# dangvansam/viet-asr

Hardware: AMD Instinct MI355X
Metric: real_time_factor (higher is better)
Workload: dtype f32 via 2xf16 split operands (22-bit significands, 3 f16 MFMA products per multiply, fp32 accumulate); 1 GPU; BASELINE configs[2]: quartznet15x5 greedy CTC, batch=64x10s 16kHz mono per GPU, wav in HBM -> collapsed ids; batch_per_gpu=64, parallelism=utterance-shard x1

## Files before the change

include/vasr_devtools.h:

```cpp
#ifndef VASR_DEVTOOLS_H_
#define VASR_DEVTOOLS_H_
#include "vasr.h"
#ifdef __cplusplus
extern "C" {
#endif

VASR_API int vasr_profile_bracket_overhead(vasr_stream stream, int n, double* out_us);
VASR_API int vasr_fused_tile_choice(int64_t tiles128, int compute_units);
VASR_API int vasr_bench_depthwise(const float* d_x, const float* d_w, const int32_t* d_lens, int batch, int channels,
                         int64_t frames, int kernel, float* d_y, vasr_stream stream);
VASR_API int vasr_bench_depthwise_layer(const float* d_x, const float* d_w, const int32_t* d_lens_in, const int32_t* d_lens_out,
                               int batch, int channels, int64_t frames_in, int kernel, int stride, int dilation, float* d_y,
                               uint32_t* d_amax, int amax_stride, vasr_stream stream);
VASR_API int vasr_depthwise_mfma_table_size(int kernel, int dilation);
VASR_API int vasr_pack_depthwise_taps(const float* h_w, int channels, int kernel, int dilation, uint32_t* h_table, float* h_inv);
VASR_API int vasr_bench_depthwise_mfma(const float* d_x, const uint32_t* d_taps, const float* d_tap_inv, const int32_t* d_lens,
                              int batch, int channels, int64_t frames, int kernel, int dilation, float* d_y,
                              uint32_t* d_amax, int amax_stride, vasr_stream stream);
VASR_API int vasr_pack_pointwise(const float* h_w, int cout, int cin, int m_pad, float* h_out);
VASR_API int vasr_conv_gemm_weights(const float* h_w, int cout, int cin, int kernel, float* h_out);
VASR_API int vasr_bench_pointwise(const float* d_x, const float* d_wt, const float* d_scale, const float* d_shift,
                         int batch, int cin, int cout, int64_t frames, float* d_y, vasr_stream stream);

VASR_API int vasr_bench_mfma_sustained(int gemm_mode, int workgroups, int steps, float* d_sink, double* flops, vasr_stream stream);

VASR_API int vasr_pack_pointwise_f16x2(const float* h_w, int cout, int cin, int m_pad, uint16_t* h_out, float* inv_scale);
VASR_API int vasr_bench_pointwise_f16x2(const float* d_x, const uint16_t* d_w16, float w_inv_scale, const float* d_scale,
                               const float* d_shift, int batch, int cin, int cout, int64_t frames, float* d_y,
                               uint32_t* d_amax, int amax_stride, vasr_stream stream);

VASR_API int vasr_pack_pointwise_bf16x3(const float* h_w, int cout, int cin, int m_pad, uint16_t* h_out);
// ... 11 lines not shown
```

viet-asr_amd/_lib.py:

```python
import ctypes as C
import os

import numpy as np
import torch

_HERE = os.path.dirname(os.path.abspath(__file__))
LIB_PATH = os.environ.get("VASR_LIB_PATH") or os.path.join(_HERE, "lib", "libvasr_hip.so")
DEV_LIB_PATH = os.environ.get("VASR_LIB_PATH") or os.path.join(_HERE, "lib", "libvasr_hip_dev.so")


class VasrError(RuntimeError):
    pass


class BlockDesc(C.Structure):
    _fields_ = [(n, C.c_int32) for n in
                ("filters", "repeat", "kernel", "stride", "dilation", "residual", "separable", "residual_dense")]


class FrontendDesc(C.Structure):
    _fields_ = [("sample_rate", C.c_int32), ("n_fft", C.c_int32), ("win_length", C.c_int32),
                ("hop_length", C.c_int32), ("n_mels", C.c_int32), ("preemph", C.c_float),
                ("log_guard", C.c_float), ("normalize", C.c_int32),
                ("h_window", C.POINTER(C.c_float)), ("h_filterbank", C.POINTER(C.c_float)),
# ... 59 lines not shown
                                 C.c_float, C.c_float, C.POINTER(_P)]),
    "vasr_lm_destroy": (None, [_P]),
    "vasr_beam_workgroups": (C.c_int, [C.c_int]),
    "vasr_beam_hash_init": (C.c_uint64, []),
    "vasr_beam_hash_step": (C.c_uint64, [C.c_uint64, C.c_uint64]),
    "vasr_last_error": (C.c_char_p, []),
    "vasr_version": (C.c_char_p, []),
    "vasr_abi_version": (C.c_int, []),
    "vasr_algorithmic_work": (C.c_int, [_P, C.c_int, C.c_int64, C.POINTER(C.c_double)]),
    "vasr_profile_begin": (C.c_int, [_P]),
    "vasr_profile_end": (C.c_int, [_P, C.POINTER(C.c_double), C.POINTER(C.c_int64), C.POINTER(C.c_double), C.POINTER(C.c_double)]),
    "vasr_padded_frames": (C.c_int64, [C.c_int64]),
}

DEV_SIGNATURES = {
    "vasr_pack_pointwise_f16x2": (C.c_int, [_P, C.c_int, C.c_int, C.c_int, _P, C.POINTER(C.c_float)]),
    "vasr_bench_pointwise_f16x2": (C.c_int, [_P, _P, C.c_float, _P, _P, C.c_int, C.c_int, C.c_int, C.c_int64, _P, _P,
                                             C.c_int, _P]),
    "vasr_depthwise_mfma_table_size": (C.c_int, [C.c_int, C.c_int]),
    "vasr_pack_depthwise_taps": (C.c_int, [_P, C.c_int, C.c_int, C.c_int, _P, _P]),
    "vasr_bench_depthwise_mfma": (C.c_int, [_P, _P, _P, _P, C.c_int, C.c_int, C.c_int64, C.c_int, C.c_int, _P, _P, C.c_int, _P]),
    "vasr_profile_bracket_overhead": (C.c_int, [_P, C.c_int, C.POINTER(C.c_double)]),
    "vasr_fused_tile_choice": (C.c_int, [C.c_int64, C.c_int]),
    "vasr_pack_pointwise": (C.c_int, [_P, C.c_int, C.c_int, C.c_int, _P]),
    "vasr_conv_gemm_weights": (C.c_int, [_P, C.c_int, C.c_int, C.c_int, _P]),
    "vasr_pack_pointwise_bf16x3": (C.c_int, [_P, C.c_int, C.c_int, C.c_int, _P]),
    "vasr_bench_pointwise_bf16x3": (C.c_int, [_P, _P, _P, _P, C.c_int, C.c_int, C.c_int, C.c_int64, _P, _P]),
    "vasr_bench_mfma_sustained": (C.c_int, [C.c_int, C.c_int, C.c_int, _P, C.POINTER(C.c_double), _P]),
    "vasr_bench_depthwise": (C.c_int, [_P, _P, _P, C.c_int, C.c_int, C.c_int64, C.c_int, _P, _P]),
    "vasr_bench_depthwise_layer": (C.c_int, [_P, _P, _P, _P, C.c_int, C.c_int, C.c_int64, C.c_int, C.c_int, C.c_int, _P, _P,
                                             C.c_int, _P]),
    "vasr_bench_pointwise": (C.c_int, [_P, _P, _P, _P, C.c_int, C.c_int, C.c_int, C.c_int64, _P, _P]),
    "vasr_bench_groupnorm": (C.c_int, [_P, _P, C.c_int, C.c_int, C.c_int64, C.c_int, C.c_int, _P, _P, C.c_int, _P, _P]),
}

ABI_VERSION = 8

_lib = None
_dev = None


def _load(path, tables):
    if not os.path.exists(path):
        raise VasrError(
            f"{path} is missing: build it with `python -c 'import __graft_entry__ as g; g.build()'` "
            "(or `make -C viet-asr_amd/csrc`). There is no CPU fallback for this path.")
# ... 167 lines not shown
```

viet-asr_amd/csrc/encoder_fused.hip:

```cpp
#include <cstdlib>

#include "vasr_internal.h"
#include "vasr_device.h"
#include <type_traits>

namespace vasr {

namespace {

constexpr int FC = 256;
constexpr int FCH = 64;
constexpr int FNT = 512;

template <int BN>
struct FTile {
  static_assert(BN == 128 || BN == 64, "tile width");
  static constexpr int FPS = BN / 8;
  static constexpr int NT = BN / 32;
  static constexpr int KHS = BN == 128 ? 3 : 2;
  static constexpr int kBimgBytes = 2 * 2 * 4 * 2 * BN * 16;
  static constexpr int kWPitch = BN == 128 ? 1664 : 1152;
  static constexpr int kWWave = 8 * kWPitch;
  static constexpr int kWinBytes = 4 * kWWave;
  static constexpr int kSegBytes = FPS * 8 + 16;
};

template <int K, int BN>
struct FGeom {
  using TL = FTile<BN>;
  static constexpr int FPS = TL::FPS;
  static constexpr int PAD = K / 2;
  static constexpr int PADL = (PAD + 3) & ~3;
  static constexpr int OFF = PADL - PAD;
  static constexpr int W = (PADL + BN + (K - 1 - PAD) + 3) & ~3;
  static constexpr int W4 = W / 4;
  static constexpr int NLD = (8 * W4 + 63) / 64;
  static constexpr int NF = OFF + FPS - 1 + K;
  static constexpr int NR = (NF + 1) / 2;
  static constexpr int KP = (K + 2) & ~1;
  static constexpr int TB = 8;
  static constexpr int NB = (K + TB - 1) / TB;
  static constexpr int kTapBytes = (FC / 2) * KP * 8;
  static constexpr size_t LDS = (size_t)TL::kBimgBytes + TL::kWinBytes + kTapBytes;
  static_assert(W * 8 + ((W + FPS - 1) / FPS) * 16 <= TL::kWPitch, "window row does not fit its pitch");
  static_assert(FPS * 7 + 2 * NR <= W, "a lane's reads leave the window");
  static_assert(NLD >= FPS / 4, "the residual rows of a lane use the staging registers of the window items");
  static_assert(LDS <= 163840, "LDS budget");
  static constexpr int qend(int blk) {
    const int k1 = TB * (blk + 1) < K ? TB * (blk + 1) : K;
    return (OFF + k1 + FPS - 1 + 1) / 2;
  }
};

struct FusedArgs {
  const float* x;
  int64_t ldx;
  const int32_t* lens_in;
  const int32_t* lens_out;
  const float* taps;
  float dw_l1;
  AmaxTab amax_x;
  const uint4* wt;
  float w_inv_scale;
  const float* scale;
  const float* shift;
  float* y;
  int64_t ldy;
  int32_t frames;
  int32_t relu;
  int32_t act;
  AmaxTab amax_y;
  const int32_t* lens_y;
  const float* x2;
  int64_t ldx2;
  const int32_t* lens2;
  AmaxTab amax_x2;
  int32_t batch;
};

__device__ __forceinline__ void lds_barrier() { asm volatile("s_waitcnt lgkmcnt(0)\n\ts_barrier" ::: "memory"); }

template <int BN>
__device__ __forceinline__ int bimg_slot(int n, int kh) { return (n & ~15) | ((n & 15) ^ ((n >> 4) | (kh << FTile<BN>::KHS))); }
template <int BN>
__device__ __forceinline__ constexpr int bimg_off(int buf, int plane, int ks) { return (((buf * 2 + plane) * 4 + ks) * 2) * BN * 16; }

template <int K, bool DUAL, int BN, int EPI = 0>
__global__ __launch_bounds__(FNT, 1) void dwpw_fused_kernel(FusedArgs a, int tiles_t, int n_blocks) {
  using G = FGeom<K, BN>;
  using TL = FTile<BN>;
  constexpr int FPS = TL::FPS, NT = TL::NT, kWPitch = TL::kWPitch, kWWave = TL::kWWave;
  extern __shared__ __attribute__((aligned(16))) unsigned char smem[];
  unsigned char* bimg = smem;
  unsigned char* wins = smem + TL::kBimgBytes;
  unsigned char* tapl = smem + TL::kBimgBytes + TL::kWinBytes;

  const int bid = xcd_remap(blockIdx.x, n_blocks);
  const int b = bid / tiles_t;
  const int tile = bid % tiles_t;
  const int t0 = tile * BN;
  const int tid = threadIdx.x, lane = tid & 63;
  const int wave = __builtin_amdgcn_readfirstlane(tid >> 6);
  const int len_in = a.lens_in[b], len_out = a.lens_out[b];
  const int len2 = DUAL ? a.lens2[b] : 0;
  constexpr int NCH = (DUAL ? 2 : 1) * (FC / FCH);

  const int zf = max(len_out, DUAL ? len2 : 0);
  const bool live = t0 < zf;

  float xs = 1.f, out_scale = 1.f;
  unsigned amv[8], amv2[8];
  if (live) {
    amax_request(a.amax_x.p, a.amax_x.stride, a.amax_x.n, b, lane, amv);
    if (DUAL) amax_request(a.amax_x2.p, a.amax_x2.stride, a.amax_x2.n, b, lane, amv2);
  }
  constexpr int kTapV4 = G::kTapBytes / 16, kTapIt = (kTapV4 + FNT - 1) / FNT;
  auto tap_copy = [&]() {
    v4f tv[kTapIt];
#pragma unroll
    for (int i = 0; i < kTapIt; ++i) {
      const int idx = tid + i * FNT;
      tv[i] = reinterpret_cast<const v4f*>(a.taps)[idx < kTapV4 ? idx : kTapV4 - 1];
    }
#pragma unroll
    for (int i = 0; i < kTapIt; ++i) {
      const int idx = tid + i * FNT;
      if (idx < kTapV4) reinterpret_cast<v4f*>(tapl)[idx] = tv[i];
    }
  };

  if (wave < 4) {
    const int kh = lane >> 5, l31 = lane & 31;
    const int wm = wave * 64;
    constexpr int ksteps = NCH * 4;
    const uint4* __restrict__ ap = a.wt + ((int64_t)(wm / 32) * ksteps) * 2 * 64 + lane;
    const int64_t a_tile = (int64_t)ksteps * 2 * 64;
    f32x16 acc[2][NT];
#pragma unroll
    for (int i = 0; i < 2; ++i)
#pragma unroll
      for (int j = 0; j < NT; ++j)
#pragma unroll
        for (int r = 0; r < 16; ++r) acc[i][j][r] = 0.f;
    if (live) {
      int boff[NT];
#pragma unroll
      for (int j = 0; j < NT; ++j) boff[j] = (kh * BN + bimg_slot<BN>(32 * j + l31, kh)) * 16;
      uint4 aw[4][2][2];
      auto aload = [&](int s, uint4 (&dst)[2][2]) {
        const int sc = s < ksteps ? s : ksteps - 1;
#pragma unroll
        for (int i = 0; i < 2; ++i)
#pragma unroll
          for (int p = 0; p < 2; ++p) dst[i][p] = ap[i * a_tile + ((int64_t)sc * 2 + p) * 64];
      };
      aload(0, aw[0]);
      aload(1, aw[1]);
      aload(2, aw[2]);
      tap_copy();
      {
        unsigned mx = amax_collect(a.amax_x.p, a.amax_x.stride, a.amax_x.n, b, lane, amv);
        mx = __float_as_uint(__uint_as_float(mx) * a.dw_l1);
        if (DUAL) mx = max(mx, amax_collect(a.amax_x2.p, a.amax_x2.stride, a.amax_x2.n, b, lane, amv2));
        float inv;
        f16_scale(mx, &xs, &inv);
        out_scale = inv * a.w_inv_scale;
      }
      lds_barrier();
#pragma unroll 1
      for (int c = 0; c < NCH; c += 2) {
#pragma unroll
        for (int cc = 0; cc < 2; ++cc) {
          lds_barrier();
          uint4 bf[3][2];
#pragma unroll
          for (int p = 0; p < 2; ++p) {
            bf[0][p] = *reinterpret_cast<const uint4*>(bimg + bimg_off<BN>(cc, p, 0) + boff[0]);
            bf[1][p] = *reinterpret_cast<const uint4*>(bimg + bimg_off<BN>(cc, p, 1 / NT) + boff[1 % NT]);
          }
#pragma unroll
          for (int s = 0; s < 4; ++s) {
            const int gs = (c + cc) * 4 + s;
            aload(gs + 3, aw[(s + 3) % 4]);
            __builtin_amdgcn_sched_barrier(0);
            uint4 (&cw)[2][2] = aw[s];
#pragma unroll
            for (int j = 0; j < NT; ++j) {
              const int g = s * NT + j, cur_f = g % 3, nxt_f = (g + 2) % 3;
              if (g + 2 < 4 * NT) {
#pragma unroll
                for (int p = 0; p < 2; ++p)
                  bf[nxt_f][p] = *reinterpret_cast<const uint4*>(bimg + bimg_off<BN>(cc, p, (g + 2) / NT) + boff[(g + 2) % NT]);
              }
              __builtin_amdgcn_sched_barrier(0);
#pragma unroll
              for (int i = 0; i < 2; ++i)
                acc[i][j] = __builtin_amdgcn_mfma_f32_32x32x16_f16(__builtin_bit_cast(f16x8, cw[i][1]), __builtin_bit_cast(f16x8, bf[cur_f][0]), acc[i][j], 0, 0, 0);
#pragma unroll
              for (int i = 0; i < 2; ++i)
                acc[i][j] = __builtin_amdgcn_mfma_f32_32x32x16_f16(__builtin_bit_cast(f16x8, cw[i][0]), __builtin_bit_cast(f16x8, bf[cur_f][1]), acc[i][j], 0, 0, 0);
#pragma unroll
              for (int i = 0; i < 2; ++i)
                acc[i][j] = __builtin_amdgcn_mfma_f32_32x32x16_f16(__builtin_bit_cast(f16x8, cw[i][0]), __builtin_bit_cast(f16x8, bf[cur_f][0]), acc[i][j], 0, 0, 0);
            }
          }
        }
      }
    }
    AmaxTracker amax{a.amax_y.p ? (a.lens_y ? a.lens_y[b] : a.frames) : 0};
    const Epilogue<EPI> epi(a.relu, a.act, 0);
    float* stage = reinterpret_cast<float*>(wins + wave * kWWave);
    v4f scv[2][4], shv[2][4];
#pragma unroll
    for (int i = 0; i < 2; ++i)
#pragma unroll
      for (int q = 0; q < 4; ++q) {
        scv[i][q] = *reinterpret_cast<const v4f*>(a.scale + wm + i * 32 + 8 * q + 4 * kh);
        shv[i][q] = *reinterpret_cast<const v4f*>(a.shift + wm + i * 32 + 8 * q + 4 * kh);
      }
#pragma unroll
    for (int i = 0; i < 2; ++i) {
#pragma unroll
      for (int q = 0; q < 4; ++q) {
        float* buf = stage + ((i * 4 + q) & 1) * (8 * BN);
        const int mq = wm + i * 32 + 8 * q;
        const v4f sc = scv[i][q], sh = shv[i][q];
        wave_fence();
#pragma unroll
        for (int rr = 0; rr < 4; ++rr)
#pragma unroll
          for (int j = 0; j < NT; ++j)
            buf[(4 * kh + rr) * BN + 32 * j + l31] = fmaf(acc[i][j][4 * q + rr] * out_scale, sc[rr], sh[rr]);
        wave_fence();
        v4f pv[NT];
#pragma unroll
        for (int k = 0; k < NT; ++k) {
          const int f = lane + 64 * k, row = f / (BN / 4), c4 = f % (BN / 4);
          pv[k] = *reinterpret_cast<const v4f*>(buf + row * BN + 4 * c4);
        }
#pragma unroll
        for (int k = 0; k < NT; ++k) {
          const int f = lane + 64 * k, row = f / (BN / 4), c4 = f % (BN / 4);
          const int m = mq + row, t = t0 + 4 * c4;
          const v4f v = epi.apply4(pv[k]);
          *reinterpret_cast<v4f*>(a.y + ((int64_t)b * FC + m) * a.ldy + t) = v;
          amax.track4(v, t);
        }
      }
    }
    if (a.amax_y.p) amax_publish(a.amax_y.p, a.amax_y.stride, b, tile * 4 + wave, amax.ymax, lane);
    return;
  }

  if (!live) return;
  const int pw = wave - 4;
  const int p = lane >> 3, s = lane & 7;
  unsigned char* win = wins + pw * kWWave;
  auto item = [&](int j, int& sp, int& q) { const int idx = lane + 64 * j; sp = idx / G::W4; q = idx - sp * G::W4; };
  v4f st[G::NLD][2];
  auto gload_dw = [&](int c) {
    const float* xb = a.x + ((int64_t)b * FC + c * FCH + pw * 16) * a.ldx;
#pragma unroll
    for (int j = 0; j < G::NLD; ++j) {
      int sp, q;
      item(j, sp, q);
      sp = sp < 8 ? sp : 7;
      int t = t0 - G::PADL + 4 * q;
      t = t < 0 ? 0 : (t > (int)a.ldx - 4 ? (int)a.ldx - 4 : t);
      const float* r0 = xb + (int64_t)(2 * sp) * a.ldx + t;
      st[j][0] = *reinterpret_cast<const v4f*>(r0);
      st[j][1] = *reinterpret_cast<const v4f*>(r0 + a.ldx);
    }
  };
  auto gload_x2 = [&](int c) {
    const float* xb = a.x2 + ((int64_t)b * FC + (c - FC / FCH) * FCH + pw * 16 + 2 * p) * a.ldx2 + t0 + FPS * s;
#pragma unroll
    for (int j = 0; j < FPS / 4; ++j) {
      st[j][0] = *reinterpret_cast<const v4f*>(xb + 4 * j);
      st[j][1] = *reinterpret_cast<const v4f*>(xb + a.ldx2 + 4 * j);
    }
  };
  gload_dw(0);
  tap_copy();
  {
    unsigned mx = amax_collect(a.amax_x.p, a.amax_x.stride, a.amax_x.n, b, lane, amv);
    mx = __float_as_uint(__uint_as_float(mx) * a.dw_l1);
    if (DUAL) mx = max(mx, amax_collect(a.amax_x2.p, a.amax_x2.stride, a.amax_x2.n, b, lane, amv2));
    float inv;
    f16_scale(mx, &xs, &inv);
  }
  lds_barrier();

  const int kh = p >> 2;
  const int wbase = (kh * BN) * 16 + 4 * (p & 3);
  const int nsw = (FPS * s) & ~15;
  const int sx = (((FPS * s) & 15) ^ (((FPS * s) >> 4) | (kh << TL::KHS))) << 4;
  auto emit = [&](int buf, const v2f (&d)[FPS], int nvalid) {
#pragma unroll
    for (int j = 0; j < FPS; ++j) {
      const float sj = j < nvalid ? xs : 0.f;
      const v2f v = {d[j].x * sj, d[j].y * sj};
      const f16x2 hv = __builtin_convertvector(v, f16x2);
      const v2f r = v - __builtin_convertvector(hv, v2f);
      const f16x2 lv = __builtin_convertvector(r, f16x2);
      const int off = wbase + ((nsw << 4) | ((j << 4) ^ sx));
      *reinterpret_cast<unsigned*>(bimg + bimg_off<BN>(buf, 0, 0) + pw * (2 * BN * 16) + off) = __builtin_bit_cast(unsigned, hv);
      *reinterpret_cast<unsigned*>(bimg + bimg_off<BN>(buf, 1, 0) + pw * (2 * BN * 16) + off) = __builtin_bit_cast(unsigned, lv);
    }
  };

  const unsigned char* rd = win + p * kWPitch + TL::kSegBytes * s;
  const int nvalid = len_out - (t0 + FPS * s);
#pragma unroll 1
  for (int c = 0; c < FC / FCH; c += 2) {
#pragma unroll
    for (int cc = 0; cc < 2; ++cc) {
      const int ch = c + cc;
#pragma unroll
      for (int j = 0; j < G::NLD; ++j) {
        int sp, q;
        item(j, sp, q);
        const int t = t0 - G::PADL + 4 * q;
        v4f u = st[j][0], w = st[j][1];
#pragma unroll
        for (int e = 0; e < 4; ++e) {
          const bool ok = (unsigned)(t + e) < (unsigned)len_in;
          u[e] = ok ? u[e] : 0.f;
          w[e] = ok ? w[e] : 0.f;
        }
        if (sp < 8) {
          unsigned char* dst = win + sp * kWPitch + (4 * q) * 8 + ((4 * q) / FPS) * 16;
          *reinterpret_cast<v4f*>(dst) = v4f{u.x, w.x, u.y, w.y};
          *reinterpret_cast<v4f*>(dst + 16) = v4f{u.z, w.z, u.w, w.w};
        }
      }
      wave_fence();
      if (ch + 1 < FC / FCH) gload_dw(ch + 1);
      else if (DUAL) gload_x2(FC / FCH);
      const unsigned char* tp = tapl + ((ch * FCH + pw * 16) / 2 + p) * (G::KP * 8);
      v2f xw[2 * G::NR];
      auto load_units = [&](int qa, int qb) {
#pragma unroll
        for (int qq = qa; qq < qb; ++qq) {
          const v4f v = *reinterpret_cast<const v4f*>(rd + qq * 16 + (qq / (FPS / 2)) * 16);
          xw[2 * qq] = v.xy;
          xw[2 * qq + 1] = v.zw;
        }
      };
      v2f acc[FPS];
#pragma unroll
      for (int j = 0; j < FPS; ++j) acc[j] = v2f{0.f, 0.f};
      load_units(0, G::qend(0));
      v2f wn[G::TB];
      auto load_taps = [&](int blk) {
#pragma unroll
        for (int k2 = 0; k2 < G::TB / 2; ++k2) {
          if (G::TB * blk + 2 * k2 < G::KP) {
            const v4f v = *reinterpret_cast<const v4f*>(tp + (G::TB * blk + 2 * k2) * 8);
            wn[2 * k2] = v.xy;
            wn[2 * k2 + 1] = v.zw;
          }
        }
// ... 21 lines not shown
      lds_barrier();
    }
  }
  if constexpr (DUAL) {
    const int nv2 = len2 - (t0 + FPS * s);
#pragma unroll 1
    for (int c = FC / FCH; c < NCH; c += 2) {
#pragma unroll
      for (int cc = 0; cc < 2; ++cc) {
        const int ch = c + cc;
        v2f d[FPS];
#pragma unroll
        for (int j = 0; j < FPS / 4; ++j)
#pragma unroll
          for (int e = 0; e < 4; ++e) d[4 * j + e] = v2f{st[j][0][e], st[j][1][e]};
        if (ch + 1 < NCH) gload_x2(ch + 1);
        emit(cc, d, nv2);
        lds_barrier();
      }
    }
  }
}

template <int K, bool DUAL, int BN>
int launch_fused_t(const FusedArgs& a, hipStream_t st, int* amax_n) {
  using G = FGeom<K, BN>;
  const int tiles_t = (int)(a.ldy / BN);
  const int n_blocks = tiles_t * a.batch;
  if (a.amax_y.p) {
    if (tiles_t * 4 > a.amax_y.stride) return (int)hipErrorInvalidValue;
    if (amax_n) *amax_n = tiles_t * 4;
  }
  const int epi = epilogue_kind(a.relu, a.act, false);
  auto kern = epi == 2 ? dwpw_fused_kernel<K, DUAL, BN, 2> : epi == 1 ? dwpw_fused_kernel<K, DUAL, BN, 1> : dwpw_fused_kernel<K, DUAL, BN, 0>;
  static std::atomic<uint64_t> lds_opted[3];
  const hipError_t attr = dyn_lds_opt_in(reinterpret_cast<const void*>(kern), (int)G::LDS, lds_opted[epi]);
  if (attr != hipSuccess) return (int)attr;
  VASR_LAUNCH(kern, dim3(n_blocks), dim3(FNT), G::LDS, st, a, tiles_t, n_blocks);
  return 0;
}

}

bool fused_dwpw_supported(int channels, int cout, int kernel, int stride, int dilation) {
  return channels == FC && cout == FC && stride == 1 && dilation == 1 && (kernel == 33 || kernel == 39);
}
int fused_dwpw_taps_per_pair(int kernel) { return (kernel + 2) & ~1; }

float pack_fused_taps(const float* w, int channels, int kernel, float* out) {
  const int kp = fused_dwpw_taps_per_pair(kernel);
  float l1 = 0.f;
  for (int c = 0; c < channels; ++c) {
    double s = 0;
    for (int k = 0; k < kernel; ++k) s += std::fabs((double)w[(size_t)c * kernel + k]);
    l1 = (float)s > l1 ? (float)s : l1;
  }
  for (int pr = 0; pr < channels / 2; ++pr)
    for (int k = 0; k < kp; ++k)
      for (int h = 0; h < 2; ++h)
        out[((size_t)pr * kp + k) * 2 + h] = k < kernel ? w[(size_t)(2 * pr + h) * kernel + k] : 0.f;
  return __builtin_nextafterf(l1, 3.0e38f);
}

int launch_fused_dwpw(const FusedLaunch& f, hipStream_t st, int* amax_n) {
  FusedArgs a{};
  a.x = f.x; a.ldx = f.ldx; a.lens_in = f.lens_in; a.lens_out = f.lens_out; a.taps = f.taps; a.dw_l1 = f.dw_l1;
  a.amax_x = f.amax_x; a.wt = reinterpret_cast<const uint4*>(f.wt); a.w_inv_scale = f.w_inv_scale; a.scale = f.scale;
  a.shift = f.shift; a.y = f.y; a.ldy = f.ldy; a.frames = f.frames; a.relu = f.relu; a.act = f.act; a.amax_y = f.amax_y;
  a.lens_y = f.lens_y; a.x2 = f.x2; a.ldx2 = f.ldx2; a.lens2 = f.lens2; a.amax_x2 = f.amax_x2; a.batch = f.batch;
  const bool dual = f.x2 != nullptr;
  if (f.tile_cols == 64) {
    if (f.kernel == 33) return dual ? launch_fused_t<33, true, 64>(a, st, amax_n) : launch_fused_t<33, false, 64>(a, st, amax_n);
    if (f.kernel == 39) return dual ? launch_fused_t<39, true, 64>(a, st, amax_n) : launch_fused_t<39, false, 64>(a, st, amax_n);
    return -1;
  }
  if (f.kernel == 33) return dual ? launch_fused_t<33, true, 128>(a, st, amax_n) : launch_fused_t<33, false, 128>(a, st, amax_n);
  if (f.kernel == 39) return dual ? launch_fused_t<39, true, 128>(a, st, amax_n) : launch_fused_t<39, false, 128>(a, st, amax_n);
  return -1;
}

}
```

viet-asr_amd/csrc/vasr_api.cpp:

```cpp
#include <hip/hip_runtime.h>

#include <cmath>
#include <cstdarg>
#include <cstdio>
#include <cstdlib>
#include <cstring>
#include <map>
#include <memory>
#include <string>
#include <algorithm>
#include <vector>

#include "vasr.h"
#include "vasr_host.h"
#include "vasr_internal.h"

using namespace vasr;

namespace {
thread_local std::string g_err;
}

namespace vasr {

// ... 960 lines not shown
      const float* gx = cur;
      int64_t gx_ld = cur_ld, g_T = cur_T;
      const int32_t* g_lens = nullptr;
      AmaxTab gx_amax = cur_amax;
      int f_cols = 0;
      const bool fuse_res = last_sub && B.fused_res;
      const ConvLayer& WF = fuse_res ? B.fused : S.pw;
      if (!h->row_independent && S.separable && S.dw.d_ftaps && h->gemm_mode == 3 && want_amax && cur_amax.p && WF.d_w16 &&
          !S.se.d_w1 && B.groups == 1 && !S.norm.d_gamma &&
          !(last_sub && B.has_res && !B.fused_res) &&
          (fuse_res ? (blk_amax.p && blk_ld == cur_ld && WF.cin == 2 * S.dw.cin && B.fused_k1 == S.dw.cin) : WF.cin == S.dw.cin) &&
          cur_ld % kTimeTile == 0 && !enc_out && (f_cols = fused_tile_cols(h, batch, cur_ld)) != 0) {
        float* dst = free3[flip];
        flip ^= 1;
        FusedLaunch f{};
        f.x = cur; f.ldx = cur_ld; f.lens_in = lens(S.dw.step); f.lens_out = lens(S.dw.step + 1);
        f.taps = S.dw.d_ftaps; f.dw_l1 = S.dw.f_l1; f.amax_x = cur_amax;
        f.wt = WF.d_w16; f.w_inv_scale = WF.w16_inv; f.scale = WF.d_scale; f.shift = WF.d_shift;
        f.y = dst; f.ldy = cur_ld; f.frames = (int)cur_T; f.relu = 1; f.act = h->act;
        f.amax_y = free_tab(cur_amax); f.lens_y = lens(S.pw.step + 1);
        if (fuse_res) { f.x2 = blk_in; f.ldx2 = blk_ld; f.lens2 = lens(B.first_step); f.amax_x2 = blk_amax; }
        f.batch = batch; f.kernel = S.dw.kernel;
        f.tile_cols = f_cols;
        int e;
        {
          ProfScope ps(h, kProfFused, st, 2.0 * WF.cin * WF.cout * (double)cur_T * batch,
                       4.0 * (2.0 + (fuse_res ? 1.0 : 0.0)) * S.dw.cin * (double)cur_T * batch);
          e = launch_fused_dwpw(f, st, &f.amax_y.n);
        }
        if (e > 0) return fail(VASR_ERR_HIP, "fused dw -> pw: %s", hipGetErrorString((hipError_t)e));
        if (e == 0) {
          cur = dst;
          cur_amax = f.amax_y;
          continue;
        }
        flip ^= 1;
      }
      if (S.separable) {
        const int64_t t_out = conv_out_frames(cur_T, S.dw);
        const int64_t ld_out = pad_frames(t_out);
        ProfScope ps(h, kProfDepthwise, st, 2.0 * S.dw.kernel * S.dw.cin * (double)t_out * batch,
                     4.0 * ((double)S.dw.cin * cur_T + (double)S.dw.cin * t_out) * batch + 4.0 * S.dw.cin * S.dw.kernel);
        AmaxTab am = want_amax ? free_tab(AmaxTab{}) : AmaxTab{};
        const bool dw_mfma = h->sw.dw_mfma;
        int e = -1;
        if (want_amax && dw_mfma && cur_amax.p && S.dw.d_taps)
// ... 936 lines not shown
```

viet-asr_amd/csrc/vasr_devtools.cpp:

```cpp
#include <hip/hip_runtime.h>

#include <algorithm>
#include <cstdio>
#include <cstdlib>
#include <initializer_list>
#include <vector>

#include "vasr.h"
#include "vasr_devtools.h"
#include "vasr_host.h"
#include "vasr_internal.h"

using namespace vasr;

const vasr::DevSwitches& vasr::dev_switches() {
  static const DevSwitches sw = [] {
    DevSwitches s;
    auto num = [](const char* name, int dflt, std::initializer_list<int> allowed) {
      const char* e = getenv(name);
      if (!e) return dflt;
      const int v = atoi(e);
      for (int a : allowed) if (a == v) return v;
      fprintf(stderr, "vasr (devtools build): %s=%s is not a documented value -- refusing to guess\n", name, e);
      abort();
      return dflt;
    };
    s.pw3_tile = num("VASR_PW3_TILE", 0, {0, 1, 2, 3, 4, 5});
    s.pw_lat = num("VASR_PW_LAT", 1, {0, 1});
    s.dw_pair = num("VASR_DW_PAIR", 1, {0, 1}) != 0;
    s.dw_mfma = num("VASR_DW_MFMA", 1, {0, 1}) != 0;
    s.dw_upw = num("VASR_DW_UPW", 0, {0, 1, 2, 3, 4, 5, 6, 7, 8});
    s.fused = num("VASR_FUSED", 1, {0, 1}) != 0;
    s.fused_min_tiles = getenv("VASR_FUSED_MIN_TILES") ? atoi(getenv("VASR_FUSED_MIN_TILES")) : 0;
    s.fused_tile = num("VASR_FUSED_TILE", 0, {0, 64, 128});
    s.fused_residual = num("VASR_NO_FUSED_RESIDUAL", 0, {0, 1}) == 0;
    s.beam_group = num("VASR_BEAM_GROUP", -1, {-1, 0, 1, 4});
    s.no_grouped = num("VASR_NO_GROUPED", 0, {0, 1}) != 0;
    return s;
  }();
  return sw;
}

extern "C" {

int vasr_fused_tile_choice(int64_t tiles128, int compute_units) { return vasr::fused_tile_choice(tiles128, compute_units); }

static __global__ void dev_noop_kernel() {}

int vasr_profile_bracket_overhead(vasr_stream stream, int n, double* out_us) {
  if (n < 1 || n > 4096 || !out_us) return fail(VASR_ERR_INVALID, "bad argument");
  hipStream_t st = static_cast<hipStream_t>(stream);
  std::vector<hipEvent_t> ev(2 * (size_t)n);
  for (auto& e : ev) HIP_TRY(hipEventCreate(&e));
  for (int i = 0; i < n; ++i) {
    HIP_TRY(hipEventRecord(ev[2 * i], st));
    hipLaunchKernelGGL(dev_noop_kernel, dim3(1), dim3(64), 0, st);
    HIP_TRY(hipEventRecord(ev[2 * i + 1], st));
  }
  HIP_TRY(hipEventSynchronize(ev.back()));
  std::vector<float> t(n);
  for (int i = 0; i < n; ++i) HIP_TRY(hipEventElapsedTime(&t[i], ev[2 * i], ev[2 * i + 1]));
  for (auto& e : ev) (void)hipEventDestroy(e);
  std::sort(t.begin(), t.end());
  *out_us = 1e3 * (double)t[n / 2];
  return 0;
}

int vasr_bench_depthwise(const float* d_x, const float* d_w, const int32_t* d_lens, int batch, int channels,
// ... 174 lines not shown
```

viet-asr_amd/csrc/vasr_internal.h:

```cpp
#pragma once
#include <hip/hip_runtime.h>
#include <atomic>
#include <hip/hip_ext.h>
#include <stdint.h>
#include <stdlib.h>

namespace vasr {

struct DevSwitches {
  int pw3_tile = 0;
  int pw_lat = 1;
  bool dw_pair = true;
  bool dw_mfma = true;
  int dw_upw = 0;
  bool fused = true;
  int fused_min_tiles = 0;
  int fused_tile = 0;
  bool fused_residual = true;
  int beam_group = -1;
  bool no_grouped = false;
};
#ifdef VASR_DEVTOOLS
const DevSwitches& dev_switches();
#else
inline const DevSwitches& dev_switches() { static constexpr DevSwitches k{}; return k; }
#endif

struct LaunchProbe { hipEvent_t start = nullptr, stop = nullptr; };
extern thread_local LaunchProbe g_probe;
#define VASR_LAUNCH(kern, grid, block, lds, st, ...)                                                       \
  do {                                                                                                     \
    if (::vasr::g_probe.start) {                                                                           \
      hipExtLaunchKernelGGL(kern, grid, block, lds, st, ::vasr::g_probe.start, ::vasr::g_probe.stop, 0,   \
                            __VA_ARGS__);                                                                  \
      ::vasr::g_probe.start = nullptr;                                                                     \
    } else {                                                                                               \
      hipLaunchKernelGGL(kern, grid, block, lds, st, __VA_ARGS__);                                         \
    }                                                                                                      \
  } while (0)

// ... 116 lines not shown
void pack_conv_gemm_weights(const float* w, int cout, int cin, int kernel, float* out);
double launch_mfma_sustained(int gemm_mode, int n_cu, int steps, float* sink, hipStream_t st);
int launch_pointwise_split(const PwArgs& a, int arith, hipStream_t st, int* amax_n = nullptr);
bool pointwise_latency_supported(int M, int K, int K1);
int launch_pointwise_latency(const PwArgs& a, hipStream_t st, int* amax_n);
int pointwise_amax_slots(int M, int64_t ld);
void pack_pointwise_weights_bf16x3(const float* w, int cout, int cin, int m_pad, unsigned short* out);
float pack_pointwise_weights_f16x2(const float* w, int cout, int cin, int m_pad, unsigned short* out);
void launch_amax(const float* x, int64_t ld, int rows, int frames, const int32_t* lens, int batch, AmaxTab* amax,
                 hipStream_t st, int64_t batch_stride = 0);

struct FusedLaunch {
  const float* x; int64_t ldx;
  const int32_t* lens_in; const int32_t* lens_out;
  const float* taps; float dw_l1;
  AmaxTab amax_x;
  const void* wt; float w_inv_scale;
  const float* scale; const float* shift;
  float* y; int64_t ldy; int32_t frames, relu, act;
  AmaxTab amax_y; const int32_t* lens_y;
  const float* x2; int64_t ldx2; const int32_t* lens2; AmaxTab amax_x2;
  int32_t batch, kernel;
  int32_t tile_cols;
};
bool fused_dwpw_supported(int channels, int cout, int kernel, int stride, int dilation);
static inline int fused_tile_choice(int64_t tiles128, int cus) {
  if (tiles128 <= 0 || cus <= 0) return 0;
  const int64_t rounds = (tiles128 + cus - 1) / cus;
  if (tiles128 >= 3 * (int64_t)cus / 4 && (double)tiles128 >= 0.8 * (double)(rounds * cus)) return 128;
  if (2 * tiles128 >= 3 * (int64_t)cus / 8 && 2 * tiles128 <= cus) return 64;
  return 0;
}
int fused_dwpw_taps_per_pair(int kernel);
float pack_fused_taps(const float* w, int channels, int kernel, float* out);
int launch_fused_dwpw(const FusedLaunch& f, hipStream_t st, int* amax_n);

struct SeLaunch {
  const float* x; float* y;
  int64_t ld, bs;
  int channels, hidden, batch, frames, store_cols;
  const int32_t* lens;
  const float* w1; const float* w2;
  float* sums; float* scale;
  const int32_t* zero_lens;
  int relu, act, accumulate;
  AmaxTab* amax_y; const int32_t* lens_y;
};
// ... 108 lines not shown
```

Before: 127,600 audio-sec/wall-sec.

## Run the fused depthwise-pointwise kernel with 16 wavefronts for 128-wide tiles

Parameterises the fused depthwise+pointwise kernel by wavefront count and, by default, launches 1024-thread workgroups for 128-column tiles. Eight MFMA waves each own one 32-row M tile instead of two, and eight producer waves each handle half a depthwise segment. The epilogue staging area is moved into the B-image and window LDS regions, and the A/B register prefetch depths are reduced. The aim is more latency hiding and more parallel depthwise production per CU, at the cost of more barrier participants, shallower per-wave pipelining and more complex LDS aliasing.

```diff
diff --git a/include/vasr_devtools.h b/include/vasr_devtools.h
--- a/include/vasr_devtools.h
+++ b/include/vasr_devtools.h
@@ -7,6 +7,7 @@
 
 VASR_API int vasr_profile_bracket_overhead(vasr_stream stream, int n, double* out_us);
 VASR_API int vasr_fused_tile_choice(int64_t tiles128, int compute_units);
+VASR_API int vasr_fused_waves_choice(int kernel, int dual, int tile_cols);
 VASR_API int vasr_bench_depthwise(const float* d_x, const float* d_w, const int32_t* d_lens, int batch, int channels,
                          int64_t frames, int kernel, float* d_y, vasr_stream stream);
 VASR_API int vasr_bench_depthwise_layer(const float* d_x, const float* d_w, const int32_t* d_lens_in, const int32_t* d_lens_out,
diff --git a/viet-asr_amd/_lib.py b/viet-asr_amd/_lib.py
--- a/viet-asr_amd/_lib.py
+++ b/viet-asr_amd/_lib.py
@@ -105,6 +105,7 @@
     "vasr_bench_depthwise_mfma": (C.c_int, [_P, _P, _P, _P, C.c_int, C.c_int, C.c_int64, C.c_int, C.c_int, _P, _P, C.c_int, _P]),
     "vasr_profile_bracket_overhead": (C.c_int, [_P, C.c_int, C.POINTER(C.c_double)]),
     "vasr_fused_tile_choice": (C.c_int, [C.c_int64, C.c_int]),
+    "vasr_fused_waves_choice": (C.c_int, [C.c_int, C.c_int, C.c_int]),
     "vasr_pack_pointwise": (C.c_int, [_P, C.c_int, C.c_int, C.c_int, _P]),
     "vasr_conv_gemm_weights": (C.c_int, [_P, C.c_int, C.c_int, C.c_int, _P]),
     "vasr_pack_pointwise_bf16x3": (C.c_int, [_P, C.c_int, C.c_int, C.c_int, _P]),
diff --git a/viet-asr_amd/csrc/encoder_fused.hip b/viet-asr_amd/csrc/encoder_fused.hip
--- a/viet-asr_amd/csrc/encoder_fused.hip
+++ b/viet-asr_amd/csrc/encoder_fused.hip
@@ -10,40 +10,46 @@
 
 constexpr int FC = 256;
 constexpr int FCH = 64;
-constexpr int FNT = 512;
-
-template <int BN>
+
+template <int BN, int NW = 8>
 struct FTile {
   static_assert(BN == 128 || BN == 64, "tile width");
-  static constexpr int FPS = BN / 8;
+  static_assert(NW == 8 || (NW == 16 && BN == 128), "wavefronts per workgroup");
+  static constexpr int NTHR = NW * 64;
+  static constexpr int NPW = NW / 2;
+  static constexpr int MT = 8 / NPW;
+  static constexpr int SEG = NW;
+  static constexpr int PP = 64 / SEG;
+  static constexpr int FPS = BN / SEG;
   static constexpr int NT = BN / 32;
   static constexpr int KHS = BN == 128 ? 3 : 2;
   static constexpr int kBimgBytes = 2 * 2 * 4 * 2 * BN * 16;
   static constexpr int kWPitch = BN == 128 ? 1664 : 1152;
-  static constexpr int kWWave = 8 * kWPitch;
-  static constexpr int kWinBytes = 4 * kWWave;
+  static constexpr int kWWave = PP * kWPitch;
+  static constexpr int kWinBytes = NPW * kWWave;
   static constexpr int kSegBytes = FPS * 8 + 16;
 };
 
-template <int K, int BN>
+template <int K, int BN, int NW = 8>
 struct FGeom {
-  using TL = FTile<BN>;
+  using TL = FTile<BN, NW>;
   static constexpr int FPS = TL::FPS;
   static constexpr int PAD = K / 2;
   static constexpr int PADL = (PAD + 3) & ~3;
   static constexpr int OFF = PADL - PAD;
   static constexpr int W = (PADL + BN + (K - 1 - PAD) + 3) & ~3;
   static constexpr int W4 = W / 4;
-  static constexpr int NLD = (8 * W4 + 63) / 64;
+  static constexpr int NLD = (TL::PP * W4 + 63) / 64;
   static constexpr int NF = OFF + FPS - 1 + K;
   static constexpr int NR = (NF + 1) / 2;
   static constexpr int KP = (K + 2) & ~1;
-  static constexpr int TB = 8;
+  static constexpr int TB = NW == 16 ? 4 : 8;
   static constexpr int NB = (K + TB - 1) / TB;
   static constexpr int kTapBytes = (FC / 2) * KP * 8;
   static constexpr size_t LDS = (size_t)TL::kBimgBytes + TL::kWinBytes + kTapBytes;
-  static_assert(W * 8 + ((W + FPS - 1) / FPS) * 16 <= TL::kWPitch, "window row does not fit its pitch");
-  static_assert(FPS * 7 + 2 * NR <= W, "a lane's reads leave the window");
+  static_assert((W - 4) * 8 + ((W - 4) / FPS) * 16 + 32 <= TL::kWPitch, "window row does not fit its pitch");
+  static_assert(FPS * (TL::SEG - 1) + 2 * NR <= W, "a lane's reads leave the window");
+  static_assert(TL::kSegBytes * (TL::SEG - 1) + (NR - 1) * 16 + ((NR - 1) / (FPS / 2)) * 16 + 16 <= TL::kWPitch, "a lane's reads leave its row");
   static_assert(NLD >= FPS / 4, "the residual rows of a lane use the staging registers of the window items");
   static_assert(LDS <= 163840, "LDS budget");
   static constexpr int qend(int blk) {
@@ -85,11 +91,15 @@
 template <int BN>
 __device__ __forceinline__ constexpr int bimg_off(int buf, int plane, int ks) { return (((buf * 2 + plane) * 4 + ks) * 2) * BN * 16; }
 
-template <int K, bool DUAL, int BN, int EPI = 0>
-__global__ __launch_bounds__(FNT, 1) void dwpw_fused_kernel(FusedArgs a, int tiles_t, int n_blocks) {
-  using G = FGeom<K, BN>;
-  using TL = FTile<BN>;
+template <int K, bool DUAL, int BN, int EPI = 0, int NW = 8>
+__global__ __launch_bounds__(NW * 64, 1) void dwpw_fused_kernel(FusedArgs a, int tiles_t, int n_blocks) {
+  using G = FGeom<K, BN, NW>;
+  using TL = FTile<BN, NW>;
   constexpr int FPS = TL::FPS, NT = TL::NT, kWPitch = TL::kWPitch, kWWave = TL::kWWave;
+  constexpr int NPW = TL::NPW, MT = TL::MT, PP = TL::PP, SEG = TL::SEG, NTHR = TL::NTHR;
+  constexpr int kStage = 2 * 8 * BN * 4;
+  static_assert(NW == 16 ? 4 * kStage <= TL::kBimgBytes / 2 && 4 * kStage <= TL::kWinBytes : kStage <= kWWave,
+                "the consumers' staging areas do not fit");
   extern __shared__ __attribute__((aligned(16))) unsigned char smem[];
   unsigned char* bimg = smem;
   unsigned char* wins = smem + TL::kBimgBytes;
@@ -114,30 +124,30 @@
     amax_request(a.amax_x.p, a.amax_x.stride, a.amax_x.n, b, lane, amv);
     if (DUAL) amax_request(a.amax_x2.p, a.amax_x2.stride, a.amax_x2.n, b, lane, amv2);
   }
-  constexpr int kTapV4 = G::kTapBytes / 16, kTapIt = (kTapV4 + FNT - 1) / FNT;
+  constexpr int kTapV4 = G::kTapBytes / 16, kTapIt = (kTapV4 + NTHR - 1) / NTHR;
   auto tap_copy = [&]() {
     v4f tv[kTapIt];
 #pragma unroll
     for (int i = 0; i < kTapIt; ++i) {
-      const int idx = tid + i * FNT;
+      const int idx = tid + i * NTHR;
       tv[i] = reinterpret_cast<const v4f*>(a.taps)[idx < kTapV4 ? idx : kTapV4 - 1];
     }
 #pragma unroll
     for (int i = 0; i < kTapIt; ++i) {
-      const int idx = tid + i * FNT;
+      const int idx = tid + i * NTHR;
       if (idx < kTapV4) reinterpret_cast<v4f*>(tapl)[idx] = tv[i];
     }
   };
 
-  if (wave < 4) {
+  if (wave < NPW) {
     const int kh = lane >> 5, l31 = lane & 31;
-    const int wm = wave * 64;
+    const int wm = wave * (32 * MT);
     constexpr int ksteps = NCH * 4;
     const uint4* __restrict__ ap = a.wt + ((int64_t)(wm / 32) * ksteps) * 2 * 64 + lane;
     const int64_t a_tile = (int64_t)ksteps * 2 * 64;
-    f32x16 acc[2][NT];
-#pragma unroll
-    for (int i = 0; i < 2; ++i)
+    f32x16 acc[MT][NT];
+#pragma unroll
+    for (int i = 0; i < MT; ++i)
 #pragma unroll
       for (int j = 0; j < NT; ++j)
 #pragma unroll
@@ -146,17 +156,18 @@
       int boff[NT];
 #pragma unroll
       for (int j = 0; j < NT; ++j) boff[j] = (kh * BN + bimg_slot<BN>(32 * j + l31, kh)) * 16;
-      uint4 aw[4][2][2];
-      auto aload = [&](int s, uint4 (&dst)[2][2]) {
+      constexpr int kAS = NW == 16 ? 2 : 4, kBS = NW == 16 ? 2 : 3, kBA = kBS - 1;
+      static_assert(4 % kAS == 0, "the set of a k-step must be a compile-time constant");
+      uint4 aw[kAS][MT][2];
+      auto aload = [&](int s, uint4 (&dst)[MT][2]) {
         const int sc = s < ksteps ? s : ksteps - 1;
 #pragma unroll
-        for (int i = 0; i < 2; ++i)
+        for (int i = 0; i < MT; ++i)
 #pragma unroll
           for (int p = 0; p < 2; ++p) dst[i][p] = ap[i * a_tile + ((int64_t)sc * 2 + p) * 64];
       };
-      aload(0, aw[0]);
-      aload(1, aw[1]);
-      aload(2, aw[2]);
+#pragma unroll
+      for (int s = 0; s < kAS - 1; ++s) aload(s, aw[s]);
       tap_copy();
       {
         unsigned mx = amax_collect(a.amax_x.p, a.amax_x.stride, a.amax_x.n, b, lane, amv);
@@ -172,35 +183,35 @@
 #pragma unroll
         for (int cc = 0; cc < 2; ++cc) {
           lds_barrier();
-          uint4 bf[3][2];
-#pragma unroll
-          for (int p = 0; p < 2; ++p) {
-            bf[0][p] = *reinterpret_cast<const uint4*>(bimg + bimg_off<BN>(cc, p, 0) + boff[0]);
-            bf[1][p] = *reinterpret_cast<const uint4*>(bimg + bimg_off<BN>(cc, p, 1 / NT) + boff[1 % NT]);
-          }
+          uint4 bf[kBS][2];
+#pragma unroll
+          for (int g0 = 0; g0 < kBA; ++g0)
+#pragma unroll
+            for (int p = 0; p < 2; ++p)
+              bf[g0][p] = *reinterpret_cast<const uint4*>(bimg + bimg_off<BN>(cc, p, g0 / NT) + boff[g0 % NT]);
 #pragma unroll
           for (int s = 0; s < 4; ++s) {
             const int gs = (c + cc) * 4 + s;
-            aload(gs + 3, aw[(s + 3) % 4]);
+            aload(gs + kAS - 1, aw[(s + kAS - 1) % kAS]);
             __builtin_amdgcn_sched_barrier(0);
-            uint4 (&cw)[2][2] = aw[s];
+            uint4 (&cw)[MT][2] = aw[s % kAS];
 #pragma unroll
             for (int j = 0; j < NT; ++j) {
-              const int g = s * NT + j, cur_f = g % 3, nxt_f = (g + 2) % 3;
-              if (g + 2 < 4 * NT) {
+              const int g = s * NT + j, cur_f = g % kBS, nxt_f = (g + kBA) % kBS;
+              if (g + kBA < 4 * NT) {
 #pragma unroll
                 for (int p = 0; p < 2; ++p)
-                  bf[nxt_f][p] = *reinterpret_cast<const uint4*>(bimg + bimg_off<BN>(cc, p, (g + 2) / NT) + boff[(g + 2) % NT]);
+                  bf[nxt_f][p] = *reinterpret_cast<const uint4*>(bimg + bimg_off<BN>(cc, p, (g + kBA) / NT) + boff[(g + kBA) % NT]);
               }
               __builtin_amdgcn_sched_barrier(0);
 #pragma unroll
-              for (int i = 0; i < 2; ++i)
+              for (int i = 0; i < MT; ++i)
                 acc[i][j] = __builtin_amdgcn_mfma_f32_32x32x16_f16(__builtin_bit_cast(f16x8, cw[i][1]), __builtin_bit_cast(f16x8, bf[cur_f][0]), acc[i][j], 0, 0, 0);
 #pragma unroll
-              for (int i = 0; i < 2; ++i)
+              for (int i = 0; i < MT; ++i)
                 acc[i][j] = __builtin_amdgcn_mfma_f32_32x32x16_f16(__builtin_bit_cast(f16x8, cw[i][0]), __builtin_bit_cast(f16x8, bf[cur_f][1]), acc[i][j], 0, 0, 0);
 #pragma unroll
-              for (int i = 0; i < 2; ++i)
+              for (int i = 0; i < MT; ++i)
                 acc[i][j] = __builtin_amdgcn_mfma_f32_32x32x16_f16(__builtin_bit_cast(f16x8, cw[i][0]), __builtin_bit_cast(f16x8, bf[cur_f][0]), acc[i][j], 0, 0, 0);
             }
           }
@@ -209,17 +220,18 @@
     }
     AmaxTracker amax{a.amax_y.p ? (a.lens_y ? a.lens_y[b] : a.frames) : 0};
     const Epilogue<EPI> epi(a.relu, a.act, 0);
-    float* stage = reinterpret_cast<float*>(wins + wave * kWWave);
-    v4f scv[2][4], shv[2][4];
-#pragma unroll
-    for (int i = 0; i < 2; ++i)
+    float* stage = reinterpret_cast<float*>(NW == 16 ? (wave < 4 ? bimg + wave * kStage : wins + (wave - 4) * kStage)
+                                                     : wins + wave * kWWave);
+    v4f scv[MT][4], shv[MT][4];
+#pragma unroll
+    for (int i = 0; i < MT; ++i)
 #pragma unroll
       for (int q = 0; q < 4; ++q) {
         scv[i][q] = *reinterpret_cast<const v4f*>(a.scale + wm + i * 32 + 8 * q + 4 * kh);
         shv[i][q] = *reinterpret_cast<const v4f*>(a.shift + wm + i * 32 + 8 * q + 4 * kh);
       }
 #pragma unroll
-    for (int i = 0; i < 2; ++i) {
+    for (int i = 0; i < MT; ++i) {
 #pragma unroll
       for (int q = 0; q < 4; ++q) {
         float* buf = stage + ((i * 4 + q) & 1) * (8 * BN);
@@ -248,36 +260,40 @@
         }
       }
     }
-    if (a.amax_y.p) amax_publish(a.amax_y.p, a.amax_y.stride, b, tile * 4 + wave, amax.ymax, lane);
+    if (a.amax_y.p) amax_publish(a.amax_y.p, a.amax_y.stride, b, tile * NPW + wave, amax.ymax, lane);
     return;
   }
 
   if (!live) return;
-  const int pw = wave - 4;
-  const int p = lane >> 3, s = lane & 7;
+  const int pw = wave - NPW;
+  const int p = lane / SEG, s = lane % SEG;
+  const int ks = NW == 16 ? pw >> 1 : pw;
+  const int kp = NW == 16 ? (pw & 1) * 4 + p : p;
   unsigned char* win = wins + pw * kWWave;
   auto item = [&](int j, int& sp, int& q) { const int idx = lane + 64 * j; sp = idx / G::W4; q = idx - sp * G::W4; };
   v4f st[G::NLD][2];
   auto gload_dw = [&](int c) {
-    const float* xb = a.x + ((int64_t)b * FC + c * FCH + pw * 16) * a.ldx;
+    const float* xb = a.x + ((int64_t)b * FC + c * FCH + pw * (2 * PP)) * a.ldx;
 #pragma unroll
     for (int j = 0; j < G::NLD; ++j) {
       int sp, q;
       item(j, sp, q);
-      sp = sp < 8 ? sp : 7;
+      sp = sp < PP ? sp : PP - 1;
       int t = t0 - G::PADL + 4 * q;
       t = t < 0 ? 0 : (t > (int)a.ldx - 4 ? (int)a.ldx - 4 : t);
-      const float* r0 = xb + (int64_t)(2 * sp) * a.ldx + t;
-      st[j][0] = *reinterpret_cast<const v4f*>(r0);
-      st[j][1] = *reinterpret_cast<const v4f*>(r0 + a.ldx);
+      const unsigned off = (unsigned)(2 * sp * (int)a.ldx + t);
+      st[j][0] = *reinterpret_cast<const v4f*>(xb + off);
+      st[j][1] = *reinterpret_cast<const v4f*>(xb + a.ldx + off);
     }
   };
   auto gload_x2 = [&](int c) {
-    const float* xb = a.x2 + ((int64_t)b * FC + (c - FC / FCH) * FCH + pw * 16 + 2 * p) * a.ldx2 + t0 + FPS * s;
+    const float* xb = a.x2 + ((int64_t)b * FC + (c - FC / FCH) * FCH + pw * (2 * PP)) * a.ldx2 + t0;
+    const float* xb1 = xb + a.ldx2;
+    const unsigned off = (unsigned)(2 * p * (int)a.ldx2 + FPS * s);
 #pragma unroll
     for (int j = 0; j < FPS / 4; ++j) {
-      st[j][0] = *reinterpret_cast<const v4f*>(xb + 4 * j);
-      st[j][1] = *reinterpret_cast<const v4f*>(xb + a.ldx2 + 4 * j);
+      st[j][0] = *reinterpret_cast<const v4f*>(xb + (off + 4 * j));
+      st[j][1] = *reinterpret_cast<const v4f*>(xb1 + (off + 4 * j));
     }
   };
   gload_dw(0);
@@ -291,11 +307,13 @@
   }
   lds_barrier();
 
-  const int kh = p >> 2;
-  const int wbase = (kh * BN) * 16 + 4 * (p & 3);
+  const int kh = kp >> 2;
+  const int wbase = (kh * BN) * 16 + 4 * (kp & 3);
   const int nsw = (FPS * s) & ~15;
   const int sx = (((FPS * s) & 15) ^ (((FPS * s) >> 4) | (kh << TL::KHS))) << 4;
   auto emit = [&](int buf, const v2f (&d)[FPS], int nvalid) {
+    int sxx = sx;
+    if constexpr (NW == 16) asm volatile("" : "+v"(nvalid), "+v"(sxx));
 #pragma unroll
     for (int j = 0; j < FPS; ++j) {
       const float sj = j < nvalid ? xs : 0.f;
@@ -303,9 +321,9 @@
       const f16x2 hv = __builtin_convertvector(v, f16x2);
       const v2f r = v - __builtin_convertvector(hv, v2f);
       const f16x2 lv = __builtin_convertvector(r, f16x2);
-      const int off = wbase + ((nsw << 4) | ((j << 4) ^ sx));
-      *reinterpret_cast<unsigned*>(bimg + bimg_off<BN>(buf, 0, 0) + pw * (2 * BN * 16) + off) = __builtin_bit_cast(unsigned, hv);
-      *reinterpret_cast<unsigned*>(bimg + bimg_off<BN>(buf, 1, 0) + pw * (2 * BN * 16) + off) = __builtin_bit_cast(unsigned, lv);
+      const int off = wbase + ((nsw << 4) | ((j << 4) ^ sxx));
+      *reinterpret_cast<unsigned*>(bimg + bimg_off<BN>(buf, 0, 0) + ks * (2 * BN * 16) + off) = __builtin_bit_cast(unsigned, hv);
+      *reinterpret_cast<unsigned*>(bimg + bimg_off<BN>(buf, 1, 0) + ks * (2 * BN * 16) + off) = __builtin_bit_cast(unsigned, lv);
     }
   };
 
@@ -328,7 +346,7 @@
           u[e] = ok ? u[e] : 0.f;
           w[e] = ok ? w[e] : 0.f;
         }
-        if (sp < 8) {
+        if (sp < PP) {
           unsigned char* dst = win + sp * kWPitch + (4 * q) * 8 + ((4 * q) / FPS) * 16;
           *reinterpret_cast<v4f*>(dst) = v4f{u.x, w.x, u.y, w.y};
           *reinterpret_cast<v4f*>(dst + 16) = v4f{u.z, w.z, u.w, w.w};
@@ -337,7 +355,7 @@
       wave_fence();
       if (ch + 1 < FC / FCH) gload_dw(ch + 1);
       else if (DUAL) gload_x2(FC / FCH);
-      const unsigned char* tp = tapl + ((ch * FCH + pw * 16) / 2 + p) * (G::KP * 8);
+      const unsigned char* tp = tapl + ((ch * FCH + pw * (2 * PP)) / 2 + p) * (G::KP * 8);
       v2f xw[2 * G::NR];
       auto load_units = [&](int qa, int qb) {
 #pragma unroll
@@ -405,24 +423,39 @@
   }
 }
 
-template <int K, bool DUAL, int BN>
+template <int K, bool DUAL, int BN, int NW = 8>
 int launch_fused_t(const FusedArgs& a, hipStream_t st, int* amax_n) {
-  using G = FGeom<K, BN>;
+  using G = FGeom<K, BN, NW>;
   const int tiles_t = (int)(a.ldy / BN);
   const int n_blocks = tiles_t * a.batch;
+  constexpr int slots = FTile<BN, NW>::NPW;
   if (a.amax_y.p) {
-    if (tiles_t * 4 > a.amax_y.stride) return (int)hipErrorInvalidValue;
-    if (amax_n) *amax_n = tiles_t * 4;
+    if (tiles_t * slots > a.amax_y.stride) return (int)hipErrorInvalidValue;
+    if (amax_n) *amax_n = tiles_t * slots;
   }
   const int epi = epilogue_kind(a.relu, a.act, false);
-  auto kern = epi == 2 ? dwpw_fused_kernel<K, DUAL, BN, 2> : epi == 1 ? dwpw_fused_kernel<K, DUAL, BN, 1> : dwpw_fused_kernel<K, DUAL, BN, 0>;
+  auto kern = epi == 2   ? dwpw_fused_kernel<K, DUAL, BN, 2, NW>
+              : epi == 1 ? dwpw_fused_kernel<K, DUAL, BN, 1, NW>
+                         : dwpw_fused_kernel<K, DUAL, BN, 0, NW>;
   static std::atomic<uint64_t> lds_opted[3];
   const hipError_t attr = dyn_lds_opt_in(reinterpret_cast<const void*>(kern), (int)G::LDS, lds_opted[epi]);
   if (attr != hipSuccess) return (int)attr;
-  VASR_LAUNCH(kern, dim3(n_blocks), dim3(FNT), G::LDS, st, a, tiles_t, n_blocks);
+  VASR_LAUNCH(kern, dim3(n_blocks), dim3(NW * 64), G::LDS, st, a, tiles_t, n_blocks);
   return 0;
 }
 
+template <int K, bool DUAL>
+int launch_fused_128(const FusedArgs& a, int waves, hipStream_t st, int* amax_n) {
+  return waves == 16 ? launch_fused_t<K, DUAL, 128, 16>(a, st, amax_n) : launch_fused_t<K, DUAL, 128, 8>(a, st, amax_n);
+}
+
+}
+
+int fused_waves_choice(int kernel, bool dual, int tile_cols, int forced) {
+  if (tile_cols == 64) return 8;
+  if (forced == 8 || forced == 16) return forced;
+  (void)kernel; (void)dual;
+  return 16;
 }
 
 bool fused_dwpw_supported(int channels, int cout, int kernel, int stride, int dilation) {
@@ -457,8 +490,9 @@
     if (f.kernel == 39) return dual ? launch_fused_t<39, true, 64>(a, st, amax_n) : launch_fused_t<39, false, 64>(a, st, amax_n);
     return -1;
   }
-  if (f.kernel == 33) return dual ? launch_fused_t<33, true, 128>(a, st, amax_n) : launch_fused_t<33, false, 128>(a, st, amax_n);
-  if (f.kernel == 39) return dual ? launch_fused_t<39, true, 128>(a, st, amax_n) : launch_fused_t<39, false, 128>(a, st, amax_n);
+  const int waves = fused_waves_choice(f.kernel, dual, 128, f.waves);
+  if (f.kernel == 33) return dual ? launch_fused_128<33, true>(a, waves, st, amax_n) : launch_fused_128<33, false>(a, waves, st, amax_n);
+  if (f.kernel == 39) return dual ? launch_fused_128<39, true>(a, waves, st, amax_n) : launch_fused_128<39, false>(a, waves, st, amax_n);
   return -1;
 }
 
diff --git a/viet-asr_amd/csrc/vasr_api.cpp b/viet-asr_amd/csrc/vasr_api.cpp
--- a/viet-asr_amd/csrc/vasr_api.cpp
+++ b/viet-asr_amd/csrc/vasr_api.cpp
@@ -1006,6 +1006,7 @@
         if (fuse_res) { f.x2 = blk_in; f.ldx2 = blk_ld; f.lens2 = lens(B.first_step); f.amax_x2 = blk_amax; }
         f.batch = batch; f.kernel = S.dw.kernel;
         f.tile_cols = f_cols;
+        f.waves = h->sw.fused_waves;
         int e;
         {
           ProfScope ps(h, kProfFused, st, 2.0 * WF.cin * WF.cout * (double)cur_T * batch,
diff --git a/viet-asr_amd/csrc/vasr_devtools.cpp b/viet-asr_amd/csrc/vasr_devtools.cpp
--- a/viet-asr_amd/csrc/vasr_devtools.cpp
+++ b/viet-asr_amd/csrc/vasr_devtools.cpp
@@ -33,6 +33,7 @@
     s.fused = num("VASR_FUSED", 1, {0, 1}) != 0;
     s.fused_min_tiles = getenv("VASR_FUSED_MIN_TILES") ? atoi(getenv("VASR_FUSED_MIN_TILES")) : 0;
     s.fused_tile = num("VASR_FUSED_TILE", 0, {0, 64, 128});
+    s.fused_waves = num("VASR_FUSED_WAVES", 0, {0, 8, 16});
     s.fused_residual = num("VASR_NO_FUSED_RESIDUAL", 0, {0, 1}) == 0;
     s.beam_group = num("VASR_BEAM_GROUP", -1, {-1, 0, 1, 4});
     s.no_grouped = num("VASR_NO_GROUPED", 0, {0, 1}) != 0;
@@ -44,6 +45,9 @@
 extern "C" {
 
 int vasr_fused_tile_choice(int64_t tiles128, int compute_units) { return vasr::fused_tile_choice(tiles128, compute_units); }
+int vasr_fused_waves_choice(int kernel, int dual, int tile_cols) {
+  return vasr::fused_waves_choice(kernel, dual != 0, tile_cols, vasr::dev_switches().fused_waves);
+}
 
 static __global__ void dev_noop_kernel() {}
 
diff --git a/viet-asr_amd/csrc/vasr_internal.h b/viet-asr_amd/csrc/vasr_internal.h
--- a/viet-asr_amd/csrc/vasr_internal.h
+++ b/viet-asr_amd/csrc/vasr_internal.h
@@ -16,6 +16,7 @@
   bool fused = true;
   int fused_min_tiles = 0;
   int fused_tile = 0;
+  int fused_waves = 0;
   bool fused_residual = true;
   int beam_group = -1;
   bool no_grouped = false;
@@ -178,7 +179,9 @@
   const float* x2; int64_t ldx2; const int32_t* lens2; AmaxTab amax_x2;
   int32_t batch, kernel;
   int32_t tile_cols;
-};
+  int32_t waves;
+};
+int fused_waves_choice(int kernel, bool dual, int tile_cols, int forced);
 bool fused_dwpw_supported(int channels, int cout, int kernel, int stride, int dilation);
 static inline int fused_tile_choice(int64_t tiles128, int cus) {
   if (tiles128 <= 0 || cus <= 0) return 0;
```

Measured after the change: 129,200 audio-sec/wall-sec (median of 6 runs). 1.01x the previous value.
